# sandyresearch/chipmunk

Hardware: AMD Instinct MI355X
Metric: DiT denoise steps/sec at fixed sparsity (higher is better)
Workload: dtype bf16

## Files before the change

### chipmunk_amd/_native.py

```python
from __future__ import annotations

import ctypes
import os

_HERE = os.path.dirname(os.path.abspath(__file__))
LIB_PATH = os.environ.get("CHIPMUNK_HIP_LIB") or os.path.join(_HERE, "lib", "libchipmunk_hip.so")

SYMBOLS = [
    "chipmunk_last_error", "chipmunk_abi_version", "chipmunk_set_option", "chipmunk_set_random_seed",
    "chipmunk_csp_attn", "chipmunk_csp_attn_out", "chipmunk_csp_128_attn", "chipmunk_dense_attn", "chipmunk_dense_colsum_attn",
    "chipmunk_csp_mlp_mm1", "chipmunk_csp_mlp_mm1_scatter", "chipmunk_csp_mlp_mm1_fp8", "chipmunk_csp_mlp_mm2_and_scatter_add", "chipmunk_csp_scatter_add", "chipmunk_csp_mlp_mm2",
    "chipmunk_csp_mlp_mm1_ragged", "chipmunk_csp_mlp_mm1_scatter_ragged", "chipmunk_csp_mlp_mm1_fp8_ragged", "chipmunk_csp_mlp_mm2_ragged",
    "chipmunk_csp_mlp_mm2_and_scatter_add_ragged", "chipmunk_csp_scatter_add_ragged", "chipmunk_block_mean_ragged", "chipmunk_transpose16_pitched",
    "chipmunk_csp_mlp_mm1_batched", "chipmunk_csp_mlp_mm1_scatter_batched", "chipmunk_csp_mlp_mm1_fp8_batched", "chipmunk_csp_mlp_mm2_batched",
    "chipmunk_csp_mlp_mm2_and_scatter_add_batched", "chipmunk_csp_scatter_add_batched",
    "chipmunk_csp_mlp_mm1_glu", "chipmunk_csp_mlp_mm1_glu_batched", "chipmunk_csp_mlp_mm1_glu_fp8", "chipmunk_csp_mlp_mm1_glu_fp8_batched",
    "chipmunk_csp_mlp_mm1_act", "chipmunk_csp_mlp_mm1_act_batched", "chipmunk_csp_mlp_mm1_fp8_act", "chipmunk_csp_mlp_mm1_fp8_act_batched",
    "chipmunk_csp_mlp_mm2_w8", "chipmunk_csp_mlp_mm2_w8_batched",
    "chipmunk_csp_mlp_mm1_w8", "chipmunk_csp_mlp_mm1_w8_batched", "chipmunk_csp_mlp_mm1_w8_gm", "chipmunk_w8_linear",
    "chipmunk_csp_mlp_mm1_fp8_act_rs", "chipmunk_csp_mlp_mm1_fp8_act_rs_batched", "chipmunk_quantize_fp8_rowwise",
    "chipmunk_csp_mlp_mm1_act_gm", "chipmunk_csp_mlp_mm1_fp8_act_gm", "chipmunk_csp_mlp_mm1_fp8_act_rs_gm", "chipmunk_csp_mlp_mm1_glu_gm",
    "chipmunk_csp_mlp_mm1_glu_fp8_gm", "chipmunk_csp_scatter_add_gm", "chipmunk_transpose16_groups",
    "chipmunk_topk_indices", "chipmunk_topk_delta_indices", "chipmunk_topk_indices_p", "chipmunk_topk_delta_indices_p", "chipmunk_topk_group_delta_indices", "chipmunk_topk_group_delta_indices_p", "chipmunk_topk_mask", "chipmunk_topk_mask_p", "chipmunk_dense_colsum_topk_mask_p_strided", "chipmunk_mask_to_indices", "chipmunk_mask_to_sorted_indices", "chipmunk_packed_mask_to_indices", "chipmunk_mask_row_counts", "chipmunk_mask_to_ragged_indices", "chipmunk_copy_indices",
    "chipmunk_bitpack", "chipmunk_bitunpack", "chipmunk_transpose16", "chipmunk_block_mean", "chipmunk_quantize_fp8", "chipmunk_gather_rows", "chipmunk_qkv_split_norm", "chipmunk_split_heads_rownorm", "chipmunk_dense_colsum_topk_mask", "chipmunk_dense_attn_strided", "chipmunk_csp_attn_out_ragged", "chipmunk_compact_indices", "chipmunk_residual_ln_modulate", "chipmunk_residual_ln_modulate_f32", "chipmunk_dense_colsum_attn_strided", "chipmunk_dense_colsum_topk_mask_strided", "chipmunk_release_scratch", "chipmunk_big_scratch_fallbacks",
    "chipmunk_dense_attn_varlen", "chipmunk_dense_colsum_attn_varlen", "chipmunk_dense_colsum_topk_mask_varlen",
    "chipmunk_dense_colsum_topk_mask_p_varlen", "chipmunk_topk_mask_varlen", "chipmunk_topk_mask_p_varlen",
    "chipmunk_host_alloc", "chipmunk_host_free", "chipmunk_copy_d2h_async", "chipmunk_copy_h2d_async", "chipmunk_host_bytes",
]

_lib = None


def lib() -> ctypes.CDLL:
    global _lib
    if _lib is None:
        if not os.path.exists(LIB_PATH):
            raise ImportError(
                f"{LIB_PATH} is missing: build it with `python -m chipmunk_amd.build` (hipcc --offload-arch=gfx950). "
                "chipmunk_amd has no CPU fallback.")
        _lib = ctypes.CDLL(LIB_PATH)
        _lib.chipmunk_last_error.restype = ctypes.c_char_p
        _lib.chipmunk_abi_version.restype = ctypes.c_int
        vp, i, d = ctypes.c_void_p, ctypes.c_int, ctypes.c_double
        if hasattr(_lib, "chipmunk_topk_group_delta_indices"):
            _lib.chipmunk_topk_group_delta_indices.argtypes = [vp, vp, i, vp, vp, i, i, i, i, d, i, d, vp]
            _lib.chipmunk_topk_group_delta_indices_p.argtypes = [vp, vp, i, vp, vp, i, i, i, i, d, d, d, i, d, vp]
        for item in filter(None, os.environ.get("CHIPMUNK_AMD_OPTIONS", "").split(",")):
            name, _, val = item.partition("=")
            if _lib.chipmunk_set_option(name.strip().encode(), int(val)) != 0:
                raise ValueError(f"CHIPMUNK_AMD_OPTIONS: {_lib.chipmunk_last_error().decode()}")
    return _lib


def last_error() -> str:
    return lib().chipmunk_last_error().decode()


def check(rc: int, what: str) -> None:
    if rc != 0:
        raise RuntimeError(f"{what}: {last_error()}")
# ... 58 lines not shown
```

### chipmunk_amd/csrc/attn64.hip

```cpp
#include "common.h"
#include "attn64_regs.h"
#include "attn_params.h"
#include "attn64_util.h"
#include <type_traits>

namespace {

constexpr int HD = 128;
constexpr int KT = 64;
constexpr int WROWS = 64, WGROWS = 256;
constexpr int TB = KT * HD * 2;
constexpr int NSL = 4;
constexpr int VRING = NSL * TB;
constexpr int LDS_BYTES = 2 * NSL * TB;
constexpr int PSTAGE = 64 * 128;
constexpr int LDS_BYTES_CSUM = LDS_BYTES + 4 * PSTAGE;
constexpr int CS_EXCH_BYTES = 2 * 4 * 64 * 4;
constexpr float SCALE_LOG2E = 0.08838834764f * 1.44269504089f;
constexpr float MAX_LAG = 4.0f;
#ifndef A64_ABL
#define A64_ABL 0
#endif
#ifndef A64_EB
#define A64_EB 20
#endif
#ifndef A64_EA
#define A64_EA 35
#endif
#ifndef A64_CSUM_VALU
#define A64_CSUM_VALU 1
#endif
#ifndef A64_VSPREAD
#define A64_VSPREAD 0
#endif
#ifndef A64_DMA_POS
#define A64_DMA_POS 2
#endif

constexpr int a64_ecum(int k) {
    return k <= 0 ? 0 : k <= 20 ? (k * A64_EB) / 20 : k <= 52 ? A64_EB + ((k - 20) * A64_EA) / 32
                                                              : (A64_EB + A64_EA + (k - 52) < 64 ? A64_EB + A64_EA + (k - 52) : 64);
}
constexpr int a64_cstep(int j) {
    int k = 0;
    while (a64_ecum(k) < 2 * j + 2) ++k;
    return k;
}
constexpr int a64_rk(int u) { return u == 0 ? 36 : u == 1 ? 38 : u == 2 ? 68 : 70; }
constexpr int a64_mk(int u) { return u == 0 ? 46 : u == 1 ? 48 : u == 2 ? 78 : 80; }

#ifdef ATTN64_PROF
__device__ unsigned long long g_a64_prof[4 * 8];
#define P64_DECL unsigned long long pt_ = 0, pacc_[7] = {0, 0, 0, 0, 0, 0, 0}; const bool prof_on_ = blockIdx.x == (gridDim.x / 2)
#define P64_START() do { if (prof_on_) pt_ = __builtin_amdgcn_s_memtime(); } while (0)
// ... 15 lines not shown
        return;
    }
    if constexpr (KS == 0)
        asm volatile("v_mfma_f32_32x32x16_bf16 %0, a[%c1:%c2], a[%c3:%c4], 0" : "=v"(s) : "i"(ka), "i"(ka + 3), "i"(qa), "i"(qa + 3));
    else
        asm volatile("v_mfma_f32_32x32x16_bf16 %0, a[%c1:%c2], a[%c3:%c4], %0" : "+v"(s) : "i"(ka), "i"(ka + 3), "i"(qa), "i"(qa + 3));
}
template <int QB, int DB>
__device__ __forceinline__ void mfma_pv(const u32x4 &vf, const u32x4 &pf) {
    constexpr int oa = (QB * 4 + DB) * 16;
    asm volatile("v_mfma_f32_32x32x16_bf16 a[%c2:%c3], %0, %1, a[%c2:%c3]" ::"v"(vf), "v"(pf), "i"(oa), "i"(oa + 15));
}
template <int KB, int KS, int SLOT>
__device__ __forceinline__ void lds_k(uint32_t addr) {
    constexpr int ka = 192 + (KB * 8 + KS) * 4;
    asm volatile("ds_read_b128 a[%c1:%c2], %0 offset:%c3" ::"v"(addr), "i"(ka), "i"(ka + 3), "i"(SLOT * TB + KB * 8192) : "memory");
}
__device__ __forceinline__ void cs_pair16x2(float &a, float &b, float &c, float &d) {
    asm volatile("v_permlane16_swap_b32 %0, %1\n\tv_permlane16_swap_b32 %2, %3\n\tv_add_f32 %0, %0, %1\n\tv_add_f32 %2, %2, %3"
                 : "+v"(a), "+v"(b), "+v"(c), "+v"(d));
}
__device__ __forceinline__ void cs_pair8(float &a, const float &b) {
    asm volatile("v_add_f32_dpp %0, %0, %0 row_mirror row_mask:0xf bank_mask:0x3\n\t"
                 "v_add_f32_dpp %0, %1, %1 row_mirror row_mask:0xf bank_mask:0xc" : "+v"(a) : "v"(b));
}
__device__ __forceinline__ void cs_pair4(float &a, const float &b) {
    asm volatile("v_add_f32_dpp %0, %0, %0 row_half_mirror row_mask:0xf bank_mask:0x5\n\t"
                 "v_add_f32_dpp %0, %1, %1 row_half_mirror row_mask:0xf bank_mask:0xa" : "+v"(a) : "v"(b));
}
template <int CTRL>
__device__ __forceinline__ float cs_pair_quad(float a, float b, bool hi) {
    const float keep = hi ? b : a, give = hi ? a : b;
    return keep + __uint_as_float((uint32_t)__builtin_amdgcn_update_dpp(0, (int)__float_as_uint(give), CTRL, 0xf, 0xf, true));
}
__global__ __launch_bounds__(256) void knorm_max_kernel(const uint16_t *k, const int64_t ks0, const int64_t ks1, const int64_t ks2, int H, int Nk,
                                                        float *out, const int32_t *klens) {
    const int bh = blockIdx.y, b = bh / H, h = bh - b * H;
    Nk = item_nk(klens, b, Nk);
    const uint16_t *kb = k + b * ks0 + h * ks1;
    const int grp = threadIdx.x >> 4, li = threadIdx.x & 15;
    float best = 0.f;
#pragma unroll 4
    for (int row = blockIdx.x * 16 + grp; row < Nk; row += gridDim.x * 16) {
        const u32x4 v = *(const u32x4 *)(kb + (int64_t)row * ks2 + li * 8);
        float ss = 0.f;
#pragma unroll
        for (int e = 0; e < 4; ++e) {
            const float lo = __uint_as_float(v[e] << 16), hi = __uint_as_float(v[e] & 0xffff0000u);
            ss = __builtin_fmaf(lo, lo, ss);
            ss = __builtin_fmaf(hi, hi, ss);
        }
        best = fmaxf(best, row16_sum(ss));
    }
    __shared__ float red[256];
    red[threadIdx.x] = best;
    __syncthreads();
    for (int st = 128; st > 0; st >>= 1) {
        if ((int)threadIdx.x < st) red[threadIdx.x] = fmaxf(red[threadIdx.x], red[threadIdx.x + st]);
        __syncthreads();
    }
    if (threadIdx.x == 0) atomicMax((unsigned int *)(out + bh), __float_as_uint(__builtin_sqrtf(red[0])));
}

template <int MODE, bool KL = false>
__global__ __launch_bounds__(256) __attribute__((amdgpu_waves_per_eu(1, 1))) void attn64_kernel(const AttnParams p) {
    static_assert(!KL || MODE == 0 || MODE == 3, "key lengths belong to the dense forms");
// ... 147 lines not shown
    auto issue_k = [&](int T, int slot) {
        const uint32_t soff = (uint32_t)tile_base(T) * kmul;
#pragma unroll
        for (int i = 0; i < 4; ++i) issue_k1(soff, w * 4096, slot, i);
    };
    auto issue_v = [&](int T, int slot) {
        const uint32_t soff = (uint32_t)tile_base(T) * vstep_b;
#pragma unroll
        for (int i = 0; i < 4; ++i) issue_v1(soff, w * 4096, slot, i);
    };

    if constexpr (!GATHER) {
        issue_k(0, 0);
        issue_k(1, 1), issue_v(0, 3);
        issue_k(2, 2), issue_v(0, 0);
        issue_k(3, 3), issue_v(1, 1);
        asm volatile("s_waitcnt vmcnt(24)" ::: "memory");
    }
    __syncthreads();
    static_for<0, 16>([&](auto i) {
        constexpr int I = decltype(i)::value;
        lds_k<(I >> 3), (I & 7), 0>(kad[I & 7]);
    });
    asm volatile("s_waitcnt lgkmcnt(0)" ::: "memory");

    f32x16 s[4];
    float px[64];
    uint32_t pw[2][4][4] = {};
    float m[2] = {-INFINITY, -INFINITY}, nmsc[2] = {0.f, 0.f};
    float mlag[2] = {-INFINITY, -INFINITY};
    float lacc[2][2] = {{0.f, 0.f}, {0.f, 0.f}};
    float alpha[2] = {1.f, 1.f};
    float wq[2] = {0.f, 0.f}, lpq[2] = {-1.0e30f, -1.0e30f}, c4[2] = {0.f, 0.f}, c5 = 0.f;
    uint32_t csoff = 0, ex_w = 0, ex_r = 0;
    int cs_extra = 0;
    float cs_own = 0.f;
    __amdgpu_buffer_rsrc_t prsrc = krsrc;
    uint32_t pst_w = 0, pst_r = 0, csoff_mx = 0;
    u32x2 csf[8] = {};
    f32x4 csacc[2] = {{0.f, 0.f, 0.f, 0.f}, {0.f, 0.f, 0.f, 0.f}};
    float csout = 0.f;
    u32x4 cs_ones = {0x3f803f80u, 0x3f803f80u, 0x3f803f80u, 0x3f803f80u};
    if constexpr (CSUM) {
        static_assert(A64_CSUM_VALU, "the matrix-pipe column-sum probe (A64_CSUM_VALU=0) fills all 160 KiB of LDS with its P stage: no room for the exchange area of the in-workgroup combine; build round 5's tree for it");
        pin(cs_ones);
        const uint32_t pst = lds0 + LDS_BYTES + (uint32_t)w * PSTAGE;
        pst_w = pst + l31 * 128 + ((uint32_t)(hf ^ (l31 & 7)) << 4);
        const int prow = lg * 4 + (l15 >> 2);
        pst_r = pst + prow * 128 + ((uint32_t)(((l15 & 3) >> 1) ^ (prow & 7)) << 4) + (l15 & 1) * 8;
        csoff_mx = 2u * (uint32_t)(16 * lg + 8 * ((l15 >> 2) & 1) + 4 * (l15 >> 3) + (l15 & 3));
        if (sub) csoff_mx = 2u * (2 * KT - 1) - csoff_mx;
#pragma unroll
        for (int qb = 0; qb < 2; ++qb) {
            const int qrow = row0 + qb * 32 + l31;
            const float pl = qrow < p.Nq ? p.p_in[(int64_t)bh * p.Nq + qrow] : 0.f;
            lpq[qb] = pl > 0.f ? __builtin_amdgcn_logf(pl) : -1.0e30f;
        }
        const int rr = ((lane >> 4) & 1) | (((lane >> 3) & 1) << 1) | (((lane >> 2) & 1) << 2);
        csoff = 2u * (uint32_t)(32 * (lane & 1) + (rr & 3) + 8 * (2 * ((lane >> 1) & 1) + (rr >> 2)) + 4 * hf);
        if (sub) csoff = 2u * (2 * KT - 1) - csoff;
        const int nA = 3 - (4 * g) % 3;
        const int lead = w < nA ? 0 : nA, members = w < nA ? nA : 4 - nA;
        cs_extra = w == lead ? members : 0;
        ex_w = lds0 + LDS_BYTES + (uint32_t)w * 256u + (uint32_t)lane * 4u;
        ex_r = lds0 + LDS_BYTES + (uint32_t)(lead + 1) * 256u + (uint32_t)lane * 4u;
        prsrc = make_rsrc(p.cs_part + ((int64_t)bh * (p.G * 2) + (g * 2 + (w < nA ? 0 : 1))) * p.cs_pstride - (sub ? KT : 0));
    }
#pragma unroll
    for (int e = 0; e < 64; ++e) px[e] = e < 20 ? 0.f : -INFINITY;

    auto vfrag_read = [&](auto dbc, auto offc) __attribute__((always_inline)) {
        constexpr int DB = decltype(dbc)::value, OFF = decltype(offc)::value;
        u32x2 lo, hi;
        asm volatile("ds_read_b64_tr_b16 %0, %2 offset:%c3\n\tds_read_b64_tr_b16 %1, %2 offset:%c4"
                     : "=&v"(lo), "=&v"(hi) : "v"(vad[DB]), "i"(OFF), "i"(OFF + 2048) : "memory");
        return (u32x4){lo[0], lo[1], hi[0], hi[1]};
    };

    static_assert(64 - A64_EB - A64_EA >= 0 && 64 - A64_EB - A64_EA <= 9, "the last steps must finish before gap 12 of the next PV phase");
    auto ecum = [](int k) constexpr { return a64_ecum(k); };
    auto finish_step = [&](auto kk, auto uwc) __attribute__((always_inline)) {
        constexpr int K = decltype(kk)::value;
        constexpr bool UW = decltype(uwc)::value != 0;
        if constexpr (!(A64_ABL & 1)) {
            static_for<ecum(K), ecum(K + 1)>([&](auto ii) {
                constexpr int I = decltype(ii)::value;
                if constexpr (A64_ABL & 32) px[I] = px[I] * 0.5f;
                else px[I] = __builtin_amdgcn_exp2f(px[I]);
                pin(px[I]);
            });
            static_for<ecum(K - 1), ecum(K)>([&](auto ii) {
                constexpr int I = decltype(ii)::value;
                lacc[(I >> 3) & 1][I & 1] += px[I];
                pin(lacc[(I >> 3) & 1][I & 1]);
            });
            static_for<(ecum(K - 1) >> 1), (ecum(K) >> 1)>([&](auto jj) {
                constexpr int J = decltype(jj)::value, I = 2 * J;
                pw[(I >> 3) & 1][I >> 4][(I & 7) >> 1] = pack_bf16x2(px[I], px[I + 1]);
                pin(pw[(I >> 3) & 1][I >> 4][(I & 7) >> 1]);
// ... 84 lines not shown
                ksoff = (uint32_t)tile_base(t + 4) * kmul;
                vsoff = (uint32_t)tile_base(t + 2) * vstep_b;
            }
        }
        __builtin_amdgcn_sched_barrier(0);
        P64_MARK(0);

        u32x4 vf[16];
        static_for<0, 32>([&](auto gg) {
            constexpr int G = decltype(gg)::value;
            constexpr int ks = G >> 2, kb = (G >> 1) & 1, qb = G & 1;
            mfma_qk<kb, qb, ks>(s[kb * 2 + qb]);
            if constexpr (!(A64_ABL & 16) && !GATHER && ((A64_DMA_POS == 0 && G < 8) || (A64_DMA_POS == 2 && G >= 16 && (G & 1) == 0))) {
                constexpr int PC = A64_DMA_POS == 0 ? G : (G - 16) >> 1;
                if constexpr (PC < 4) issue_k1(ksoff, ldsw, SL, PC);
                else issue_v1(vsoff, ldsw, (SL + 2) & 3, PC - 4);
            }
            finish_step(ic<20 + G>{}, uwc);
            if constexpr (A64_VSPREAD ? (G & 1) == 0 : G < 16) {
                constexpr int f = A64_VSPREAD ? G >> 1 : G;
                if constexpr (A64_ABL & 4) vf[f] = (u32x4){(uint32_t)t, 1u, 2u, 3u};
                else vf[f] = vfrag_read(ic<(f & 3)>{}, ic<VSL * TB + (f >> 2) * 4096>{});
            }
            __builtin_amdgcn_sched_barrier(0);
        });
        P64_MARK(1);
        asm volatile("s_waitcnt lgkmcnt(0)"
                     : "+v"(vf[0]), "+v"(vf[1]), "+v"(vf[2]), "+v"(vf[3]), "+v"(vf[4]), "+v"(vf[5]), "+v"(vf[6]), "+v"(vf[7]), "+v"(vf[8]),
                       "+v"(vf[9]), "+v"(vf[10]), "+v"(vf[11]), "+v"(vf[12]), "+v"(vf[13]), "+v"(vf[14]), "+v"(vf[15]));
        __builtin_amdgcn_sched_barrier(0);
        P64_MARK(2);

        float mx[2];
        bool moved = false;
        const int dead = GATHER ? 0 : (t * KT - tile_base(t) + dadj < KT ? t * KT - tile_base(t) + dadj : KT);
        const int vleft = !GATHER ? KT : (t < ntiles ? valid - (tbeg + t) * KT : 0);
        auto phase_b_gap = [&](auto gg) __attribute__((always_inline)) {
            constexpr int G = decltype(gg)::value;
            constexpr int up = G >> 3, db = (G >> 1) & 3, qb = G & 1;
            const u32x4 pf = {pw[qb][up][0], pw[qb][up][1], pw[qb][up][2], pw[qb][up][3]};
            mfma_pv<qb, db>(vf[G >> 1], pf);
            constexpr bool UWT = decltype(uwc)::value != 0 && !A64_CSUM_VALU;
            if constexpr (G < (CSUM ? (UWT ? 32 : 17) : 12)) finish_step(ic<52 + G>{}, uwc);
            if constexpr (CSUM && G == (UWT ? 31 : 17)) {
                const uint32_t par2 = (uint32_t)(t & 1) * 1024u;
                const float mine = UWT ? csout : c5;
                if (!cs_extra) {
                    asm volatile("ds_write_b32 %0, %1" ::"v"(ex_w + (par2 ^ 1024u)), "v"(mine) : "memory");
                } else {
                    float x1 = 0.f, x2 = 0.f;
                    if (cs_extra >= 2) asm volatile("ds_read_b32 %0, %1" : "=v"(x1) : "v"(ex_r + par2) : "memory");
                    if (cs_extra >= 3) asm volatile("ds_read_b32 %0, %1 offset:256" : "=v"(x2) : "v"(ex_r + par2) : "memory");
                    asm volatile("ds_write_b32 %0, %1" ::"v"(ex_w + (par2 ^ 1024u)), "v"(mine) : "memory");
                    asm volatile("s_waitcnt lgkmcnt(1)" : "+v"(x1), "+v"(x2)::"memory");
                    const int tb2 = tile_base(t - 2), dd = (t - 2) * KT - tb2;
                    if (t > 1 && dd < KT) {
                        const uint32_t off = UWT ? csoff_mx : csoff;
                        if (dd <= 0 || (int)(off >> 1) >= dd) {
                            const uint16_t val = (uint16_t)(pack_bf16x2((cs_own + x1) + x2, 0.f) & 0xffffu);
                            if (p.probe & 16) __builtin_amdgcn_raw_buffer_store_b16(val, prsrc, off, (uint32_t)(KL && tb2 < 0 ? 0 : tb2) * 2u, 2);
                            else __builtin_amdgcn_raw_buffer_store_b16(val, prsrc, off, (uint32_t)(KL && tb2 < 0 ? 0 : tb2) * 2u, 0);
                        }
                    }
                }
                cs_own = mine;
            }
            if constexpr (!(A64_ABL & 16) && !GATHER && A64_DMA_POS == 1 && G >= 16 && (G & 1) == 0) {
                constexpr int PC = (G - 16) >> 1;
                if constexpr (PC < 4) issue_k1(ksoff, ldsw, SL, PC);
                else issue_v1(vsoff, ldsw, (SL + 2) & 3, PC - 4);
            }
            if constexpr (G < 16 && !(A64_ABL & 8)) {
                constexpr int J = G;
                lds_k<(J >> 3), (J & 7), KNSL>(kad[J & 7]);
            }
            if constexpr (G == 1 && !(A64_ABL & 2)) {
                if (!GATHER && __builtin_expect(dead > 0, 0)) {
                    int thr = dead - 4 * hf;
                    asm volatile("" : "+v"(thr));
#pragma unroll
                    for (int blk = 0; blk < 4; ++blk)
#pragma unroll
                        for (int r = 0; r < 16; ++r)
                            if ((blk >> 1) * 32 + (r & 3) + 8 * (r >> 2) < thr) s[blk][r] = -INFINITY;
                }
                if (GATHER && __builtin_expect(vleft < KT, 0)) {
                    int thr = vleft - hf;
                    asm volatile("" : "+v"(thr));
#pragma unroll
                    for (int blk = 0; blk < 4; ++blk)
#pragma unroll
                        for (int r = 0; r < 16; ++r)
                            if ((r & 3) * 16 + (blk >> 1) * 8 + 2 * (r >> 2) >= thr) s[blk][r] = -INFINITY;
                }
            }
            if constexpr (G >= 2 && G <= 9 && !(A64_ABL & 2) && !NOMAX) {
                constexpr int j = G - 2;
// ... 100 lines not shown
    if (CSUM && unitw) {
        if constexpr (CSUM) {
            for (int tb = 0;; tb += 4) {
                tile(ic<0>{}, ic<2>{}, tb);
                if (tb >= T4) break;
                tile(ic<1>{}, ic<2>{}, tb + 1);
                tile(ic<2>{}, ic<2>{}, tb + 2);
                tile(ic<3>{}, ic<2>{}, tb + 3);
            }
        }
    } else if (nomax) {
        for (int tb = 0;; tb += 4) {
            tile(ic<0>{}, ic<1>{}, tb);
            if (tb >= T4) break;
            tile(ic<1>{}, ic<1>{}, tb + 1);
            tile(ic<2>{}, ic<1>{}, tb + 2);
            tile(ic<3>{}, ic<1>{}, tb + 3);
        }
    } else {
        for (int tb = 0;; tb += 4) {
            tile(ic<0>{}, ic<0>{}, tb);
            if (tb >= T4) break;
            tile(ic<1>{}, ic<0>{}, tb + 1);
            tile(ic<2>{}, ic<0>{}, tb + 2);
            tile(ic<3>{}, ic<0>{}, tb + 3);
        }
    }
    asm volatile("s_waitcnt vmcnt(0)" ::: "memory");
    P64_END(w, T4 + 1);
    if constexpr (CSUM) {
        asm volatile("s_waitcnt lgkmcnt(0)" ::: "memory");
        __builtin_amdgcn_s_barrier();
        if (cs_extra) {
            float x1 = 0.f, x2 = 0.f;
            const uint32_t par = (uint32_t)((T4 - 1) & 1) * 1024u;
            if (cs_extra >= 2) asm volatile("ds_read_b32 %0, %1" : "=v"(x1) : "v"(ex_r + par) : "memory");
            if (cs_extra >= 3) asm volatile("ds_read_b32 %0, %1 offset:256" : "=v"(x2) : "v"(ex_r + par) : "memory");
            asm volatile("s_waitcnt lgkmcnt(0)" : "+v"(x1), "+v"(x2)::"memory");
            const int tb1 = tile_base(T4 - 1), dd = (T4 - 1) * KT - tb1;
            const uint32_t off = (unitw && !A64_CSUM_VALU) ? csoff_mx : csoff;
            if (dd < KT && (dd <= 0 || (int)(off >> 1) >= dd))
                __builtin_amdgcn_raw_buffer_store_b16((uint16_t)(pack_bf16x2((cs_own + x1) + x2, 0.f) & 0xffffu), prsrc, off, (uint32_t)(KL && tb1 < 0 ? 0 : tb1) * 2u, 0);
        }
    }

    asm volatile("s_nop 7\n\ts_nop 7\n\ts_nop 7" ::: "memory");
    float o[128];
    static_for<0, 32>([&](auto ii) {
        constexpr int I = decltype(ii)::value;
        const f32x4 o4 = acc_read4<I * 4>();
        o[I * 4 + 0] = o4[0], o[I * 4 + 1] = o4[1], o[I * 4 + 2] = o4[2], o[I * 4 + 3] = o4[3];
    });
    float lq[2];
#pragma unroll
    for (int qb = 0; qb < 2; ++qb) {
        float lp = lacc[qb][0] + lacc[qb][1], lo2 = lp;
        lane_swap32(lp, lo2);
        lq[qb] = lp + lo2;
    }

    if constexpr (GATHER) {
        if (nsp > 1) {
            constexpr int SLICE_FLOATS = 26 * 256 * 4;
            int *ticket_s = (int *)smem;
            float *mine = p.ws + (int64_t)(slot0 + sp) * SLICE_FLOATS + tid;
#pragma unroll
            for (int i = 0; i < 128; ++i) mine[i * 192] = o[i];
            mine[128 * 192] = m[0], mine[129 * 192] = m[1], mine[130 * 192] = lq[0], mine[131 * 192] = lq[1];
            __syncthreads();
            if (tid == 0) {
                __builtin_amdgcn_fence(__ATOMIC_RELEASE, "agent");
                asm volatile("s_waitcnt vmcnt(0)" ::: "memory");
                *ticket_s = __hip_atomic_fetch_add(p.tickets + tix, 1, __ATOMIC_RELAXED, __HIP_MEMORY_SCOPE_AGENT);
            }
            __syncthreads();
// ... 288 lines not shown
            if (j >= Nk) return;
            if (KL && j >= nv) {
                dst[j] = 0;
                continue;
            }
            float acc = bf16_bits_to_f32(src[j]);
            if (nrows == 2) acc += bf16_bits_to_f32(src[row1 + j]);
            dst[j] = f32_to_bf16_bits(acc);
        }
    }
}
}

int chipmunk_colsum64_launch(const AttnParams &p, hipStream_t stream) {
    static uint64_t lds_set = 0;
    ensure_dynamic_lds((const void *)colsum64_kernel, NSL * TB, lds_set);
    const int64_t grid = (int64_t)p.B * p.H * ((p.G + 3) / 4);
    hipLaunchKernelGGL(colsum64_kernel, dim3((unsigned)grid), dim3(256), NSL * TB, stream, p);
    CM_LAUNCH_CHECK();
    return CHIPMUNK_OK;
}

int chipmunk_colsum_part_stride(int Nk) { return (chipmunk_get_option("attn_cs_probe") & 1) ? Nk : (Nk + 63) & ~63; }

size_t chipmunk_colsum_part_bytes(int B, int H, int Nq, int Nk) {
    return (size_t)B * H * (((Nq + WGROWS - 1) / WGROWS) * 2) * (size_t)chipmunk_colsum_part_stride(Nk) * sizeof(uint16_t);
}

int chipmunk_dense64_colsum_launch(const AttnParams &p0, uint16_t *part, hipStream_t stream) {
    AttnParams p = p0;
    const int G192 = p.G;
    p.G = (p.Nq + WGROWS - 1) / WGROWS;
    p.cs_part = part, p.cs_pstride = chipmunk_colsum_part_stride(p.Nk);
    if (chipmunk_get_option("attn_cs_probe") & 2) p.probe |= 16;
    if (chipmunk_get_option("attn_fused_colsum") == 3) p.probe |= 4;
    p.kmax = chipmunk_knorm_max(p.k, p.ks, p.B, p.H, p.Nk, stream, p.klens);
    if (int rc = p.klens ? launch64<3, true>(p, (int64_t)p.B * p.H * p.G, stream) : launch64<3>(p, (int64_t)p.B * p.H * p.G, stream)) return rc;
    if (!p.cs) return CHIPMUNK_OK;
    const dim3 cgrid((unsigned)((p.Nk + 1023) / 1024), (unsigned)G192, (unsigned)(p.B * p.H));
    if (p.klens)
        hipLaunchKernelGGL(cs_combine_kernel<true>, cgrid, dim3(256), 0, stream, part, p.cs_pstride, p.cs, p.G * 2, G192, p.Nq, p.Nk, p.cs_stride,
                           p.klens, p.H);
    else
        hipLaunchKernelGGL(cs_combine_kernel<false>, cgrid, dim3(256), 0, stream, part, p.cs_pstride, p.cs, p.G * 2, G192, p.Nq, p.Nk, p.cs_stride,
                           p.klens, p.H);
    CM_LAUNCH_CHECK();
    return CHIPMUNK_OK;
}

int chipmunk_csp64_launch(const AttnParams &p, int inplace, int grid, hipStream_t stream) {
    CM_CHECK(p.plan && p.tickets && p.ws, "csp64: work plan missing");
    return inplace ? launch64<2>(p, grid, stream) : launch64<1>(p, grid, stream);
}
```

### chipmunk_amd/csrc/capi.hip

```cpp
#include "common.h"

static thread_local char g_last_error[512] = "";

void chipmunk_set_error(const char *fmt, ...) {
    va_list ap;
    va_start(ap, fmt);
    vsnprintf(g_last_error, sizeof(g_last_error), fmt, ap);
    va_end(ap);
}

extern "C" const char *chipmunk_last_error(void) { return g_last_error; }
extern "C" int chipmunk_abi_version(void) { return 1; }

#include <string.h>
namespace {
struct Option { const char *name; int value; };
Option g_options[] = {{"mm1_variant", 0}, {"mm2_variant", 0}, {"attn_variant", 0}, {"m2i_variant", 0}, {"topk_variant", 0}, {"mm1_nr", 0}, {"mm2_nr", 0}, {"mm1_probe", 0}, {"attn_xcd_chunks", 0}, {"attn_no_order", 0}, {"attn_no_tail", 0}, {"mm1_no_split", 0}, {"mm2_no_split", 0}, {"attn_no_split", 0}, {"attn_split_gather", 0}, {"attn_pp", 0}, {"attn_dense64", 0}, {"attn_csp64", 0}, {"attn_colsum64", 0}, {"attn_csp96", 0}, {"attn_nomax", 0}, {"attn_fused_colsum", 0}, {"attn_cs_probe", 0}, {"big_scratch_gb", 0}, {"attn_balanced", 0}, {"attn_row_split", 0}, {"mm2_order", 0}, {"topk_mask_stream", 0}};
}
int chipmunk_get_option(const char *name) {
    for (auto &o : g_options) if (strcmp(o.name, name) == 0) return o.value;
    return 0;
}
extern "C" int chipmunk_set_option(const char *name, int value) {
    for (auto &o : g_options) if (strcmp(o.name, name) == 0) { o.value = value; return CHIPMUNK_OK; }
// ... 67 lines not shown
    if (want > cap) return ++g_big_fallbacks, nullptr;
    size_t free_b = 0, total_b = 0;
    const bool have_info = hipMemGetInfo(&free_b, &total_b) == hipSuccess;
    auto f = g_big_failed.find(dev);
    if (f != g_big_failed.end() && want >= f->second.want) {
        const bool more_free = have_info && free_b > f->second.free_then + ((size_t)1 << 30);
        if (!more_free && --f->second.calls_left > 0) return ++g_big_fallbacks, nullptr;
        g_big_failed.erase(f);
        f = g_big_failed.end();
    }
    auto failed = [&]() {
        g_big_failed[dev] = BigFail{f == g_big_failed.end() ? want : std::min(f->second.want, want), free_b, 64};
        ++g_big_fallbacks;
        return nullptr;
    };
    if (have_info && want > free_b + s.bytes - std::min(free_b + s.bytes, (size_t)4 << 30)) return failed();
    if (s.ptr) {
        (void)hipStreamSynchronize(stream);
        (void)hipFree(s.ptr);
        s.ptr = nullptr, s.bytes = 0;
    }
    void *ptr = nullptr;
    if (hipMalloc(&ptr, want) != hipSuccess) {
        (void)hipGetLastError();
        return failed();
    }
    s.ptr = ptr, s.bytes = want;
    return ptr;
}
extern "C" int chipmunk_big_scratch_fallbacks(void) {
    std::lock_guard<std::mutex> lock(g_scratch_mu);
    return g_big_fallbacks;
}
namespace {
std::mutex g_host_mu;
std::map<void *, size_t> g_host_allocs;
size_t g_host_total = 0;
}
extern "C" int chipmunk_host_alloc(size_t bytes, void **host_ptr) {
    CM_CHECK(host_ptr != nullptr && bytes > 0, "chipmunk_host_alloc: null result pointer or zero bytes");
    void *p = nullptr;
    const hipError_t e = hipHostMalloc(&p, bytes, hipHostMallocDefault);
    if (e != hipSuccess || !p) {
        chipmunk_set_error("chipmunk_host_alloc: hipHostMalloc(%zu) failed: %s", bytes, hipGetErrorString(e));
        return CHIPMUNK_ERR_LAUNCH;
    }
    std::lock_guard<std::mutex> lock(g_host_mu);
    g_host_allocs[p] = bytes;
    g_host_total += bytes;
    *host_ptr = p;
    return CHIPMUNK_OK;
}
extern "C" int chipmunk_host_free(void *host_ptr) {
    if (!host_ptr) return CHIPMUNK_OK;
    {
        std::lock_guard<std::mutex> lock(g_host_mu);
        auto it = g_host_allocs.find(host_ptr);
        CM_CHECK(it != g_host_allocs.end(), "chipmunk_host_free: %p was not allocated by chipmunk_host_alloc", host_ptr);
        g_host_total -= it->second;
        g_host_allocs.erase(it);
    }
    (void)hipHostFree(host_ptr);
    return CHIPMUNK_OK;
}
extern "C" size_t chipmunk_host_bytes(void) {
    std::lock_guard<std::mutex> lock(g_host_mu);
// ... 33 lines not shown
```

### include/chipmunk_hip.h

```cpp
#ifndef CHIPMUNK_HIP_H
#define CHIPMUNK_HIP_H

#include <stdint.h>

#ifdef __cplusplus
extern "C" {
#endif

#define CHIPMUNK_OK 0
#define CHIPMUNK_ERR_INVALID 1
#define CHIPMUNK_ERR_LAUNCH 2
#define CHIPMUNK_ERR_UNSUPPORTED 3

#define CHIPMUNK_DTYPE_BF16 0
#define CHIPMUNK_DTYPE_FP16 1
#define CHIPMUNK_DTYPE_FP32 2

const char *chipmunk_last_error(void);
int chipmunk_abi_version(void);
int chipmunk_set_option(const char *name, int value);
int chipmunk_set_random_seed(uint64_t seed);

int chipmunk_csp_attn(const void *q, const void *k, const void *v, void *o, const int64_t q_strides[3],
                      const int64_t k_strides[3], const int64_t v_strides[3], const int64_t o_strides[3],
// ... 261 lines not shown
int chipmunk_mask_row_counts(const void *mask, int packed, int32_t *counts, int64_t *lengths, int64_t rows, int n, int pad_n,
                             int multiple_of, void *stream);
int chipmunk_mask_to_ragged_indices(const void *mask, int packed, int sorted, const int64_t *offsets, int32_t *flat, int64_t rows,
                                    int n, int multiple_of, void *stream);

int chipmunk_copy_indices(const void *src, void *dst, const int32_t *inds, const int32_t *counts, int B, int M, int R,
                          int F, int elem_size, void *stream);

int chipmunk_transpose16(const void *src, void *dst, int B, int R, int C, void *stream);
int chipmunk_transpose16_pitched(const void *src, void *dst, int B, int R, int C, int ld, void *stream);

int chipmunk_block_mean(const void *x, void *out, int64_t rows, int C, int mbm, void *stream);
int chipmunk_block_mean_ragged(const void *x, void *out, int64_t rows, int C, int mbm, void *stream);

int chipmunk_quantize_fp8(const void *x, const float *scale, void *out, int64_t n, float max_value, void *stream);

#define CHIPMUNK_QUANTIZE_ROWWISE_MAX_K 16384
int chipmunk_quantize_fp8_rowwise(const void *x, void *out, float *scale_recip, int64_t rows, int K, float max_value, void *stream);

int chipmunk_bitpack(const void *mask, void *packed, int64_t n, void *stream);
int chipmunk_bitunpack(const void *packed, void *mask, int64_t n, void *stream);

int chipmunk_gather_rows(const void *src, void *dst, const int32_t *map, int64_t outer, int64_t n_src, int64_t n_out,
                         int64_t row_bytes, void *stream);

int chipmunk_host_alloc(size_t bytes, void **host_ptr);
int chipmunk_host_free(void *host_ptr);
int chipmunk_copy_d2h_async(void *host_dst, const void *dev_src, size_t bytes, void *stream);
int chipmunk_copy_h2d_async(void *dev_dst, const void *host_src, size_t bytes, void *stream);
size_t chipmunk_host_bytes(void);

int chipmunk_release_scratch(void);
int chipmunk_big_scratch_fallbacks(void);

int chipmunk_qkv_split_norm(const void *qkv, int64_t row_stride, const void *q_weight, const void *k_weight, void *q, void *k,
                            void *v, int64_t n, int heads, float eps, const float *freqs_cos, const float *freqs_sin,
                            int64_t rope_rows, void *stream);

int chipmunk_split_heads_rownorm(const void *x, int64_t batch_stride, int64_t row_stride, int parts, const void *w0, int w0_dtype,
                                 const void *w1, int w1_dtype, const void *w2, int w2_dtype, void *out0, void *out1, void *out2,
                                 unsigned norm_mask, unsigned rope_mask, int64_t B, int64_t n, int heads, float eps,
                                 const float *freqs_cos, const float *freqs_sin, int64_t rope_rows, void *stream);

#ifdef __cplusplus
}
#endif
#endif
```

Before: 0.5926.

## Make fused colsum cross-wave exchange branch-free with early LDS reads and bounded stores

Reworks the column-sum partial exchange in the fused dense attention kernel. The lead wave's data-dependent branch at the exchange step is removed. All waves now issue the two LDS reads earlier in the PV loop and wait with a counted lgkmcnt, and they store through a bounds-checked buffer resource whose out-of-range offsets drop the write instead of a conditional branch. This aims to hide LDS latency and cut wave divergence. The costs are extra stores from non-lead waves, which are dropped via the offset, and a zeroed dummy exchange slot. It also adds a debug helper for copying big scratch memory and removes the probe option.

```diff
diff --git a/chipmunk_amd/_native.py b/chipmunk_amd/_native.py
--- a/chipmunk_amd/_native.py
+++ b/chipmunk_amd/_native.py
@@ -25,7 +25,7 @@
     "chipmunk_bitpack", "chipmunk_bitunpack", "chipmunk_transpose16", "chipmunk_block_mean", "chipmunk_quantize_fp8", "chipmunk_gather_rows", "chipmunk_qkv_split_norm", "chipmunk_split_heads_rownorm", "chipmunk_dense_colsum_topk_mask", "chipmunk_dense_attn_strided", "chipmunk_csp_attn_out_ragged", "chipmunk_compact_indices", "chipmunk_residual_ln_modulate", "chipmunk_residual_ln_modulate_f32", "chipmunk_dense_colsum_attn_strided", "chipmunk_dense_colsum_topk_mask_strided", "chipmunk_release_scratch", "chipmunk_big_scratch_fallbacks",
     "chipmunk_dense_attn_varlen", "chipmunk_dense_colsum_attn_varlen", "chipmunk_dense_colsum_topk_mask_varlen",
     "chipmunk_dense_colsum_topk_mask_p_varlen", "chipmunk_topk_mask_varlen", "chipmunk_topk_mask_p_varlen",
-    "chipmunk_host_alloc", "chipmunk_host_free", "chipmunk_copy_d2h_async", "chipmunk_copy_h2d_async", "chipmunk_host_bytes",
+    "chipmunk_host_alloc", "chipmunk_host_free", "chipmunk_copy_d2h_async", "chipmunk_copy_h2d_async", "chipmunk_host_bytes", "chipmunk_big_scratch_copy",
 ]
 
 _lib = None
diff --git a/chipmunk_amd/csrc/attn64.hip b/chipmunk_amd/csrc/attn64.hip
--- a/chipmunk_amd/csrc/attn64.hip
+++ b/chipmunk_amd/csrc/attn64.hip
@@ -15,11 +15,17 @@
 constexpr int LDS_BYTES = 2 * NSL * TB;
 constexpr int PSTAGE = 64 * 128;
 constexpr int LDS_BYTES_CSUM = LDS_BYTES + 4 * PSTAGE;
-constexpr int CS_EXCH_BYTES = 2 * 4 * 64 * 4;
+constexpr int CS_EXCH_PAR = 5 * 64 * 4;
+constexpr int CS_EXCH_BYTES = 2 * CS_EXCH_PAR;
+constexpr int CS_RD_GAP = 12;
+constexpr uint32_t CS_DROP = 0x40000000u;
 constexpr float SCALE_LOG2E = 0.08838834764f * 1.44269504089f;
 constexpr float MAX_LAG = 4.0f;
 #ifndef A64_ABL
 #define A64_ABL 0
+#endif
+#ifndef A64_CS_UNIFORM
+#define A64_CS_UNIFORM 1
 #endif
 #ifndef A64_EB
 #define A64_EB 20
@@ -101,6 +107,12 @@
 __device__ __forceinline__ float cs_pair_quad(float a, float b, bool hi) {
     const float keep = hi ? b : a, give = hi ? a : b;
     return keep + __uint_as_float((uint32_t)__builtin_amdgcn_update_dpp(0, (int)__float_as_uint(give), CTRL, 0xf, 0xf, true));
+}
+__device__ __forceinline__ void cs_store(__amdgpu_buffer_rsrc_t prsrc, uint32_t lb128, uint32_t end128, uint32_t u128, float sum, uint32_t off) {
+    const bool live = u128 < end128;
+    const int rag = (int)(lb128 - u128);
+    const uint32_t adj = live ? (uint32_t)(rag < 0 ? rag : 0) : CS_DROP;
+    __builtin_amdgcn_raw_buffer_store_b16((uint16_t)(pack_bf16x2(sum, 0.f) & 0xffffu), prsrc, off + adj, live ? u128 : 0u, 0);
 }
 __global__ __launch_bounds__(256) void knorm_max_kernel(const uint16_t *k, const int64_t ks0, const int64_t ks1, const int64_t ks2, int H, int Nk,
                                                         float *out, const int32_t *klens) {
@@ -314,7 +326,8 @@
     float lacc[2][2] = {{0.f, 0.f}, {0.f, 0.f}};
     float alpha[2] = {1.f, 1.f};
     float wq[2] = {0.f, 0.f}, lpq[2] = {-1.0e30f, -1.0e30f}, c4[2] = {0.f, 0.f}, c5 = 0.f;
-    uint32_t csoff = 0, ex_w = 0, ex_r = 0;
+    uint32_t csoff = 0, ex_w = 0, ex_r1 = 0, ex_r2 = 0;
+    uint32_t cs_lb128 = 0, cs_end128 = 0;
     int cs_extra = 0;
     float cs_own = 0.f;
     __amdgpu_buffer_rsrc_t prsrc = krsrc;
@@ -331,7 +344,7 @@
         const int prow = lg * 4 + (l15 >> 2);
         pst_r = pst + prow * 128 + ((uint32_t)(((l15 & 3) >> 1) ^ (prow & 7)) << 4) + (l15 & 1) * 8;
         csoff_mx = 2u * (uint32_t)(16 * lg + 8 * ((l15 >> 2) & 1) + 4 * (l15 >> 3) + (l15 & 3));
-        if (sub) csoff_mx = 2u * (2 * KT - 1) - csoff_mx;
+        if (sub) csoff_mx = 2u * (KT - 1) - csoff_mx;
 #pragma unroll
         for (int qb = 0; qb < 2; ++qb) {
             const int qrow = row0 + qb * 32 + l31;
@@ -340,13 +353,20 @@
         }
         const int rr = ((lane >> 4) & 1) | (((lane >> 3) & 1) << 1) | (((lane >> 2) & 1) << 2);
         csoff = 2u * (uint32_t)(32 * (lane & 1) + (rr & 3) + 8 * (2 * ((lane >> 1) & 1) + (rr >> 2)) + 4 * hf);
-        if (sub) csoff = 2u * (2 * KT - 1) - csoff;
+        if (sub) csoff = 2u * (KT - 1) - csoff;
         const int nA = 3 - (4 * g) % 3;
         const int lead = w < nA ? 0 : nA, members = w < nA ? nA : 4 - nA;
         cs_extra = w == lead ? members : 0;
-        ex_w = lds0 + LDS_BYTES + (uint32_t)w * 256u + (uint32_t)lane * 4u;
-        ex_r = lds0 + LDS_BYTES + (uint32_t)(lead + 1) * 256u + (uint32_t)lane * 4u;
-        prsrc = make_rsrc(p.cs_part + ((int64_t)bh * (p.G * 2) + (g * 2 + (w < nA ? 0 : 1))) * p.cs_pstride - (sub ? KT : 0));
+        const uint32_t ex0 = lds0 + LDS_BYTES + (uint32_t)lane * 4u;
+        ex_w = ex0 + (uint32_t)w * 256u;
+        ex_r1 = ex0 + (uint32_t)(members >= 2 ? lead + 1 : 4) * 256u;
+        ex_r2 = ex0 + (uint32_t)(members >= 3 ? lead + 2 : 4) * 256u;
+        if (w < 2) asm volatile("ds_write_b32 %0, %1" ::"v"(ex0 + 4 * 256u + (uint32_t)w * CS_EXCH_PAR), "v"(0.f) : "memory");
+        asm volatile("s_waitcnt lgkmcnt(0)" ::: "memory");
+        const int ncol = sub ? KT : valid;
+        prsrc = make_rsrc(p.cs_part + ((int64_t)bh * (p.G * 2) + (g * 2 + (w < nA ? 0 : 1))) * p.cs_pstride, (uint32_t)ncol * 2u);
+        cs_lb128 = (uint32_t)(ncol - KT) * 2u;
+        cs_end128 = cs_extra ? (uint32_t)ntiles * (2u * KT) : 0u;
     }
 #pragma unroll
     for (int e = 0; e < 64; ++e) px[e] = e < 20 ? 0.f : -INFINITY;
@@ -497,6 +517,7 @@
         P64_MARK(2);
 
         float mx[2];
+        float csx[2] = {0.f, 0.f};
         bool moved = false;
         const int dead = GATHER ? 0 : (t * KT - tile_base(t) + dadj < KT ? t * KT - tile_base(t) + dadj : KT);
         const int vleft = !GATHER ? KT : (t < ntiles ? valid - (tbeg + t) * KT : 0);
@@ -507,27 +528,17 @@
             mfma_pv<qb, db>(vf[G >> 1], pf);
             constexpr bool UWT = decltype(uwc)::value != 0 && !A64_CSUM_VALU;
             if constexpr (G < (CSUM ? (UWT ? 32 : 17) : 12)) finish_step(ic<52 + G>{}, uwc);
-            if constexpr (CSUM && G == (UWT ? 31 : 17)) {
-                const uint32_t par2 = (uint32_t)(t & 1) * 1024u;
+            constexpr int CSG = UWT ? 31 : 17, CSR = UWT ? 30 : CS_RD_GAP;
+            if constexpr (CSUM && G == CSR && !(A64_ABL & 512))
+                asm volatile("ds_read_b32 %0, %2 offset:%c4\n\tds_read_b32 %1, %3 offset:%c4"
+                             : "=&v"(csx[0]), "=&v"(csx[1]) : "v"(ex_r1), "v"(ex_r2), "i"((SL & 1) * CS_EXCH_PAR) : "memory");
+            if constexpr (CSUM && G == CSG) {
                 const float mine = UWT ? csout : c5;
-                if (!cs_extra) {
-                    asm volatile("ds_write_b32 %0, %1" ::"v"(ex_w + (par2 ^ 1024u)), "v"(mine) : "memory");
-                } else {
-                    float x1 = 0.f, x2 = 0.f;
-                    if (cs_extra >= 2) asm volatile("ds_read_b32 %0, %1" : "=v"(x1) : "v"(ex_r + par2) : "memory");
-                    if (cs_extra >= 3) asm volatile("ds_read_b32 %0, %1 offset:256" : "=v"(x2) : "v"(ex_r + par2) : "memory");
-                    asm volatile("ds_write_b32 %0, %1" ::"v"(ex_w + (par2 ^ 1024u)), "v"(mine) : "memory");
-                    asm volatile("s_waitcnt lgkmcnt(1)" : "+v"(x1), "+v"(x2)::"memory");
-                    const int tb2 = tile_base(t - 2), dd = (t - 2) * KT - tb2;
-                    if (t > 1 && dd < KT) {
-                        const uint32_t off = UWT ? csoff_mx : csoff;
-                        if (dd <= 0 || (int)(off >> 1) >= dd) {
-                            const uint16_t val = (uint16_t)(pack_bf16x2((cs_own + x1) + x2, 0.f) & 0xffffu);
-                            if (p.probe & 16) __builtin_amdgcn_raw_buffer_store_b16(val, prsrc, off, (uint32_t)(KL && tb2 < 0 ? 0 : tb2) * 2u, 2);
-                            else __builtin_amdgcn_raw_buffer_store_b16(val, prsrc, off, (uint32_t)(KL && tb2 < 0 ? 0 : tb2) * 2u, 0);
-                        }
-                    }
-                }
+                asm volatile("ds_write_b32 %0, %1 offset:%c2" ::"v"(ex_w), "v"(mine), "i"(((SL & 1) ^ 1) * CS_EXCH_PAR) : "memory");
+                constexpr int YOUNGER = 1 + ((A64_ABL & 8) || CSR >= 16 ? 0 : 16 - CSR);
+                if constexpr (!(A64_ABL & 512)) asm volatile("s_waitcnt lgkmcnt(%c2)" : "+v"(csx[0]), "+v"(csx[1]) : "i"(YOUNGER) : "memory");
+                if constexpr (!(A64_ABL & 1024))
+                    if (A64_CS_UNIFORM || cs_extra) cs_store(prsrc, cs_lb128, cs_end128, (uint32_t)(t - 2) * (2u * KT), (cs_own + csx[0]) + csx[1], UWT ? csoff_mx : csoff);
                 cs_own = mine;
             }
             if constexpr (!(A64_ABL & 16) && !GATHER && A64_DMA_POS == 1 && G >= 16 && (G & 1) == 0) {
@@ -694,15 +705,10 @@
         asm volatile("s_waitcnt lgkmcnt(0)" ::: "memory");
         __builtin_amdgcn_s_barrier();
         if (cs_extra) {
-            float x1 = 0.f, x2 = 0.f;
-            const uint32_t par = (uint32_t)((T4 - 1) & 1) * 1024u;
-            if (cs_extra >= 2) asm volatile("ds_read_b32 %0, %1" : "=v"(x1) : "v"(ex_r + par) : "memory");
-            if (cs_extra >= 3) asm volatile("ds_read_b32 %0, %1 offset:256" : "=v"(x2) : "v"(ex_r + par) : "memory");
-            asm volatile("s_waitcnt lgkmcnt(0)" : "+v"(x1), "+v"(x2)::"memory");
-            const int tb1 = tile_base(T4 - 1), dd = (T4 - 1) * KT - tb1;
-            const uint32_t off = (unitw && !A64_CSUM_VALU) ? csoff_mx : csoff;
-            if (dd < KT && (dd <= 0 || (int)(off >> 1) >= dd))
-                __builtin_amdgcn_raw_buffer_store_b16((uint16_t)(pack_bf16x2((cs_own + x1) + x2, 0.f) & 0xffffu), prsrc, off, (uint32_t)(KL && tb1 < 0 ? 0 : tb1) * 2u, 0);
+            float x1, x2;
+            const uint32_t par = (uint32_t)((T4 - 1) & 1) * CS_EXCH_PAR;
+            asm volatile("ds_read_b32 %0, %2\n\tds_read_b32 %1, %3\n\ts_waitcnt lgkmcnt(0)" : "=&v"(x1), "=&v"(x2) : "v"(ex_r1 + par), "v"(ex_r2 + par) : "memory");
+            cs_store(prsrc, cs_lb128, cs_end128, (uint32_t)(T4 - 1) * (2u * KT), (cs_own + x1) + x2, (unitw && !A64_CSUM_VALU) ? csoff_mx : csoff);
         }
     }
 
@@ -1057,7 +1063,6 @@
     const int G192 = p.G;
     p.G = (p.Nq + WGROWS - 1) / WGROWS;
     p.cs_part = part, p.cs_pstride = chipmunk_colsum_part_stride(p.Nk);
-    if (chipmunk_get_option("attn_cs_probe") & 2) p.probe |= 16;
     if (chipmunk_get_option("attn_fused_colsum") == 3) p.probe |= 4;
     p.kmax = chipmunk_knorm_max(p.k, p.ks, p.B, p.H, p.Nk, stream, p.klens);
     if (int rc = p.klens ? launch64<3, true>(p, (int64_t)p.B * p.H * p.G, stream) : launch64<3>(p, (int64_t)p.B * p.H * p.G, stream)) return rc;
diff --git a/chipmunk_amd/csrc/capi.hip b/chipmunk_amd/csrc/capi.hip
--- a/chipmunk_amd/csrc/capi.hip
+++ b/chipmunk_amd/csrc/capi.hip
@@ -123,6 +123,25 @@
     std::lock_guard<std::mutex> lock(g_scratch_mu);
     return g_big_fallbacks;
 }
+extern "C" int chipmunk_big_scratch_copy(void *buf, size_t offset, size_t bytes, int to_scratch, size_t *size, void *stream) {
+    int dev = 0;
+    CM_CHECK(hipGetDevice(&dev) == hipSuccess, "big_scratch_copy: no device");
+    Scratch s = {nullptr, 0};
+    {
+        std::lock_guard<std::mutex> lock(g_scratch_mu);
+        auto it = g_big.find({dev, (hipStream_t)stream});
+        if (it != g_big.end()) s = it->second;
+    }
+    if (size) *size = s.bytes;
+    if (bytes == 0) return CHIPMUNK_OK;
+    CM_CHECK(buf != nullptr, "big_scratch_copy: null buffer");
+    CM_CHECK(s.ptr != nullptr && offset <= s.bytes && bytes <= s.bytes - offset, "big_scratch_copy: bytes [%zu, +%zu) are not inside the %zu-byte scratch",
+             offset, bytes, s.bytes);
+    unsigned char *sp = (unsigned char *)s.ptr + offset;
+    CM_CHECK(hipMemcpyAsync(to_scratch ? (void *)sp : buf, to_scratch ? buf : (void *)sp, bytes, hipMemcpyDeviceToDevice, (hipStream_t)stream) == hipSuccess,
+             "big_scratch_copy: copy failed");
+    return CHIPMUNK_OK;
+}
 namespace {
 std::mutex g_host_mu;
 std::map<void *, size_t> g_host_allocs;
diff --git a/include/chipmunk_hip.h b/include/chipmunk_hip.h
--- a/include/chipmunk_hip.h
+++ b/include/chipmunk_hip.h
@@ -317,6 +317,7 @@
 
 int chipmunk_release_scratch(void);
 int chipmunk_big_scratch_fallbacks(void);
+int chipmunk_big_scratch_copy(void *buf, size_t offset, size_t bytes, int to_scratch, size_t *size, void *stream);
 
 int chipmunk_qkv_split_norm(const void *qkv, int64_t row_stride, const void *q_weight, const void *k_weight, void *q, void *k,
                             void *v, int64_t n, int heads, float eps, const float *freqs_cos, const float *freqs_sin,
```

Result: no change. 0.5922 (median of 2 runs) (-0.1%).
